# InternLM/lmdeploy

Measured on AMD Instinct MI355X. Metric: decode tokens/sec, Llama-3-8B W4A16 int8-KV batch 64 (1024-in/1k-out synthetic), higher is better.
Workload: dtype f16

## Files before the change

lmdeploy_amd/csrc/gemm_decode_lc.hip:

```cpp
#include "gemm_decode_common.h"
#include <stdlib.h>

namespace tmk {

typedef float floatx2 __attribute__((ext_vector_type(2)));

__device__ __forceinline__ half8_t raw8_p32(uint32_t w)
{
    const uint32_t m = 0x000f000fu;
    return bit_cast<half8_t>(u32x4{w & m, (w >> 4) & m, (w >> 8) & m, (w >> 12) & m});
}

template<int MH, int PFS, int ABL = 0>
__global__ __launch_bounds__(768) void gemm_dec_lc_kernel(Dec32Params p)
{
    constexpr int NCW   = 2;
    constexpr int CGW   = 2;
    constexpr int WK    = 4;
    constexpr int NCONS = CGW * WK;
    constexpr int NLOAD = 4;
    constexpr int T     = (NCONS + NLOAD) * 64;
    constexpr int ROWS  = 32 * MH;
    constexpr int KBB   = ROWS * 256;
    constexpr int S     = WK;
    constexpr int STG   = S * KBB;
    constexpr int CGT   = CGW * NCW;
    constexpr int NPC   = S * ROWS / 4;
    constexpr int DR    = NPC / NLOAD;
    static_assert(NPC % NLOAD == 0, "DMA pieces per loader wave");
    static_assert(WK * ROWS * CGT * 128 <= 2 * STG, "reduction image must fit the stage buffers");

    extern __shared__ __attribute__((aligned(16))) char smem[];

    const int tid  = threadIdx.x;
    const int wgid = blockIdx.y * gridDim.x + blockIdx.x;
    if (p.dbg && tid == 0) {
        p.dbg[wgid * 8 + 0] = __builtin_amdgcn_s_memrealtime();
        p.dbg[wgid * 8 + 4] = ((uint64_t)__builtin_amdgcn_s_getreg(20 | (31 << 11)) << 32) | (uint32_t)__builtin_amdgcn_s_getreg(4 | (31 << 11));
    }
    const int lane = tid & 63;
    const int wave = __builtin_amdgcn_readfirstlane(tid >> 6);
    const int l31  = lane & 31;
    const int half = lane >> 5;

    const int kb0 = blockIdx.y * p.kb_per_split;
    const int nkb = min(p.kb_per_split, p.KB - kb0);
    const int nst = (nkb + S - 1) / S;
    const int Mloc = min(ROWS, p.M);

    const unsigned lds0 = __builtin_amdgcn_readfirstlane((unsigned)(size_t)smem);

    floatx16 acc[NCW][MH];
#pragma unroll
    for (int c = 0; c < NCW; ++c) {
#pragma unroll
        for (int h = 0; h < MH; ++h) {
#pragma unroll
            for (int r = 0; r < 16; ++r) {
                acc[c][h][r] = 0.f;
            }
        }
    }
    const int cw = wave & (CGW - 1);
    const int wk = wave / CGW;

    if (wave >= NCONS) {
        const int  lw   = wave - NCONS;
        const auto rs_x = __builtin_amdgcn_make_buffer_rsrc((void*)p.x, 0, (int)(((size_t)(Mloc - 1) * p.ldx + p.K) * 2), 0x00020000);
        int        doff[DR];
#pragma unroll
        for (int r = 0; r < DR; ++r) {
            const int pc  = r * NLOAD + lw;
            const int kbi = pc / (ROWS / 4);
            const int row = (pc % (ROWS / 4)) * 4 + (lane >> 4);
            const int ch  = (lane & 15) ^ (row & 15);
            doff[r]       = (ABL & 0x20) ? (kbi * ROWS + row) * 256 + ch * 16
                                          : (min(row, Mloc - 1) * p.ldx + ch * 8) * 2 + kbi * 256;
        }
#define LC_DMA_X(t, buf)                                                                                          \
    _Pragma("unroll") for (int r = 0; r < DR; ++r)                                                                \
    {                                                                                                             \
        unsigned       keep_;                                                                                     \
        const unsigned dst_ = lds0 + (buf)*STG + (r * NLOAD + lw) * 1024;                                         \
        const int      so_  = (kb0 + (t)*S) * ((ABL & 0x20) ? ROWS * 256 : 256);                                  \
        asm volatile("s_mov_b32 %0, m0\n\ts_mov_b32 m0, %3\n\ts_nop 0\n\t"                                       \
                     "buffer_load_dwordx4 %1, %2, %4 offen lds\n\ts_mov_b32 m0, %0"                               \
                     : "=&s"(keep_)                                                                               \
                     : "v"(doff[r]), "s"(rs_x), "s"(dst_), "s"(so_)                                               \
                     : "memory");                                                                                 \
    }
        if (nst > 0) {
            if constexpr (!(ABL & 8)) {
                LC_DMA_X(0, 0);
            }
            asm volatile("s_waitcnt vmcnt(0)" ::: "memory");
            __builtin_amdgcn_s_barrier();
            for (int t = 0; t < nst; ++t) {
                if constexpr (!(ABL & 8)) {
                    if (t + 1 < nst) {
                        LC_DMA_X(t + 1, (t + 1) & 1);
                    }
                }
                asm volatile("s_waitcnt vmcnt(0)" ::: "memory");
                __builtin_amdgcn_s_barrier();
            }
        }
#undef LC_DMA_X
    }
    else {
        int cgc[NCW];
#pragma unroll
        for (int c = 0; c < NCW; ++c) {
            cgc[c] = min((int)blockIdx.x * CGT + cw * NCW + c, p.ncg - 1);
        }
        const auto rs_w = __builtin_amdgcn_make_buffer_rsrc((void*)p.wp, 0, (int)((size_t)p.KB * p.ncg * kP32Unit), 0x00020000);
        const int  vw   = lane * 16;
        const int  vs   = 2048 + l31 * 4;
        u32x4      ring[PFS][NCW][2];
        uint32_t   sring[PFS][NCW];
        const int frow = l31 * 256;
        const int fsw  = (half ^ (l31 & 15)) << 4;
        uint32_t  m1024 = 0x64006400u, m64 = 0x54005400u;
        asm volatile("" : "+v"(m1024), "+v"(m64));

#define LC_LOAD_W(slot, b)                                                                                        \
    _Pragma("unroll") for (int c = 0; c < NCW; ++c)                                                               \
    {                                                                                                             \
        const int uo_      = ((kb0 + min((b), nkb - 1)) * p.ncg + cgc[c]) * kP32Unit;                             \
        ring[slot][c][0]   = __builtin_amdgcn_raw_buffer_load_b128(rs_w, vw, uo_,  2);                      \
        ring[slot][c][1]   = __builtin_amdgcn_raw_buffer_load_b128(rs_w, vw + 1024, uo_,  2);               \
        sring[slot][c]     = __builtin_amdgcn_raw_buffer_load_b32(rs_w, vs, uo_, 0);                              \
    }
        if (nst > 0) {
#pragma unroll
            for (int u = 0; u < PFS; ++u) {
                if constexpr (!(ABL & 16)) {
                    LC_LOAD_W(u, u * S + wk);
                }
                __builtin_amdgcn_sched_barrier(0);
            }
            __builtin_amdgcn_s_barrier();
            if (p.dbg && tid == 0) {
                p.dbg[wgid * 8 + 1] = __builtin_amdgcn_s_memrealtime();
                p.dbg[wgid * 8 + 5] = __builtin_amdgcn_s_memtime();
            }
            auto stage = [&](auto U, const int t) __attribute__((always_inline)) {
                constexpr int u    = decltype(U)::value;
                const int     b    = t * S + wk;
                const bool    live = b < nkb;
                half2_t       s2[NCW], z2[NCW];
#pragma unroll
                for (int c = 0; c < NCW; ++c) {
                    const half2_t pr = bit_cast<half2_t>(live ? sring[u][c] : 0u);
                    s2[c]            = half2_t{pr[0], pr[0]};
                    z2[c]            = half2_t{pr[1], pr[1]};
                }
                half8_t        f0[MH], f1[MH];
                const unsigned xa = lds0 + (t & 1) * STG + wk * KBB;
                auto           rd = [&](half8_t(&f)[MH], int j) __attribute__((always_inline)) {
                    const unsigned ad = xa + (unsigned)(frow + ((32 * j) ^ fsw));
#pragma unroll
                    for (int h = 0; h < MH; ++h) {
                        asm volatile("ds_read_b128 %0, %1 offset:%2" : "=v"(f[h]) : "v"(ad), "i"(h * 8192));
                    }
                };
                auto wt = [&](half8_t(&f)[MH], auto N) __attribute__((always_inline)) {
                    constexpr int n = decltype(N)::value;
                    if constexpr (MH == 1) {
                        asm volatile("s_waitcnt lgkmcnt(%1)" : "+v"(f[0]) : "i"(n));
                    }
                    else {
                        asm volatile("s_waitcnt lgkmcnt(%2)" : "+v"(f[0]), "+v"(f[1]) : "i"(n));
                    }
                    __builtin_amdgcn_sched_barrier(0);
                };
                if constexpr (!(ABL & 4)) {
                    rd(f0, 0);
                }
                half8_t a0 = (ABL & 0x40) ? raw8_p32(ring[u][0][0][0]) : dequant8_p32(ring[u][0][0][0], s2[0], z2[0], m1024, m64), a1;
                if constexpr (ABL & 0x80) {
#pragma unroll
                    for (int c = 0; c < NCW; ++c) {
                        const float   rt = 1.0f + (float)s2[c][0];
                        const floatx2 rr = {rt, rt};
#pragma unroll
                        for (int h = 0; h < MH; ++h) {
#pragma unroll
                            for (int r = 0; r < 8; ++r) {
                                floatx2 v        = {acc[c][h][2 * r], acc[c][h][2 * r + 1]};
                                v                = v * rr;
                                acc[c][h][2 * r] = v[0], acc[c][h][2 * r + 1] = v[1];
                            }
                        }
                    }
                }
                static_for<8>([&](auto J) {
                    constexpr int  j  = decltype(J)::value;
                    half8_t(&cur)[MH] = (j & 1) ? f1 : f0;
                    half8_t(&nxt)[MH] = (j & 1) ? f0 : f1;
                    if constexpr (!(ABL & 4)) {
                        if constexpr (j + 1 < 8) {
                            rd(nxt, j + 1);
                        }
                        wt(cur, std::integral_constant<int, (j + 1 < 8) ? MH : 0>{});
                    }
                    else {
#pragma unroll
                        for (int h = 0; h < MH; ++h) {
                            cur[h] = bit_cast<half8_t>(ring[u][h & 1][1]);
                        }
                    }
                    if constexpr (ABL & 1) {
                        a1 = bit_cast<half8_t>(ring[u][1][j >> 2]);
                    }
                    else if constexpr (ABL & 0x40) {
                        a1 = raw8_p32(ring[u][1][j >> 2][j & 3]);
                    }
                    else {
                        a1 = dequant8_p32(ring[u][1][j >> 2][j & 3], s2[1], z2[1], m1024, m64);
                    }
#pragma unroll
                    for (int h = 0; h < MH; ++h) {
                        if constexpr (ABL & 2) {
                            asm volatile("" ::"v"(a0), "v"(cur[h]));
                        }
                        else {
                            acc[0][h] = __builtin_amdgcn_mfma_f32_32x32x16_f16(a0, cur[h], acc[0][h], 0, 0, 0);
                        }
                    }
                    if constexpr (j + 1 < 8) {
                        if constexpr (ABL & 1) {
                            a0 = bit_cast<half8_t>(ring[u][0][(j + 1) >> 2]);
                        }
                        else if constexpr (ABL & 0x40) {
                            a0 = raw8_p32(ring[u][0][(j + 1) >> 2][(j + 1) & 3]);
                        }
                        else {
                            a0 = dequant8_p32(ring[u][0][(j + 1) >> 2][(j + 1) & 3], s2[0], z2[0], m1024, m64);
                        }
                    }
#pragma unroll
                    for (int h = 0; h < MH; ++h) {
                        if constexpr (ABL & 2) {
                            asm volatile("" ::"v"(a1), "v"(cur[h]));
                        }
                        else {
                            acc[1][h] = __builtin_amdgcn_mfma_f32_32x32x16_f16(a1, cur[h], acc[1][h], 0, 0, 0);
                        }
                    }
                    if constexpr (!(ABL & (1 | 2))) {
#pragma unroll
                        for (int g = 0; g < 2 * MH; ++g) {
                            __builtin_amdgcn_sched_group_barrier(0x008, 1, 0);
                            __builtin_amdgcn_sched_group_barrier(0x002, MH == 2 ? 7 : 14, 0);
                        }
                    }
                    __builtin_amdgcn_sched_barrier(0);
                });
                if constexpr (!(ABL & 16)) {
                    LC_LOAD_W(u, (t + PFS) * S + wk);
                }
                __builtin_amdgcn_s_barrier();
            };
            int t0 = 0;
            for (; t0 + PFS <= nst; t0 += PFS) {
                static_for<PFS>([&](auto U) { stage(U, t0 + decltype(U)::value); });
            }
            static_for<PFS>([&](auto U) {
                if (t0 + decltype(U)::value < nst) {
                    stage(U, t0 + decltype(U)::value);
                }
            });
        }
#undef LC_LOAD_W
    }
    if (p.dbg && tid == 0) {
        p.dbg[wgid * 8 + 2] = __builtin_amdgcn_s_memrealtime();
        p.dbg[wgid * 8 + 6] = __builtin_amdgcn_s_memtime();
    }

    {
        constexpr int C4  = CGT * 8;
        floatx4*      red = (floatx4*)smem;
        if (wave < NCONS) {
#pragma unroll
            for (int c = 0; c < NCW; ++c) {
#pragma unroll
                for (int h = 0; h < MH; ++h) {
                    const int m = 32 * h + l31;
#pragma unroll
                    for (int g4 = 0; g4 < 4; ++g4) {
                        const int c4 = (cw * NCW + c) * 8 + 2 * g4 + half;
                        red[(wk * ROWS + m) * C4 + (c4 ^ (m & 7))] =
                            floatx4{acc[c][h][4 * g4], acc[c][h][4 * g4 + 1], acc[c][h][4 * g4 + 2], acc[c][h][4 * g4 + 3]};
                    }
                }
            }
        }
        __syncthreads();
        if (p.dbg && tid == 0) {
            p.dbg[wgid * 8 + 7] = __builtin_amdgcn_s_memrealtime();
        }
        constexpr int NE    = ROWS * C4;
        const int     ncol0 = blockIdx.x * CGT * 32;
#pragma unroll
        for (int e0 = 0; e0 < NE; e0 += T) {
            const int e = e0 + tid;
            if (NE % T != 0 && e >= NE) {
                break;
            }
            const int m  = e / C4;
            const int c4 = e % C4;
            floatx4   a  = red[m * C4 + (c4 ^ (m & 7))];
#pragma unroll
            for (int k = 1; k < WK; ++k) {
                a += red[(k * ROWS + m) * C4 + (c4 ^ (m & 7))];
            }
            const int n = ncol0 + c4 * 4;
            if (m >= Mloc || n >= p.N) {
                continue;
            }
            if (p.epilogue == 2) {
                floatx4* dst = (floatx4*)(p.partial + ((size_t)blockIdx.y * p.M + m) * p.N + n);
                if (p.wt & 1) {
                    store_wt(dst, a, p.wt >> 4);
                }
                else {
                    *dst = a;
                }
            }
            else if (p.epilogue == 1) {
                const float s0 = a[0] / (1.0f + __builtin_expf(-a[0]));
                const float s1 = a[2] / (1.0f + __builtin_expf(-a[2]));
                half2_t     o  = {(half_t)(s0 * a[1]), (half_t)(s1 * a[3])};
                half2_t*    dst = (half2_t*)(p.y + (size_t)m * p.ldy + (n >> 1));
                if (p.wt & 2) {
                    store_wt(dst, o);
                }
                else {
                    *dst = o;
                }
            }
            else {
                half4_t  o   = {(half_t)a[0], (half_t)a[1], (half_t)a[2], (half_t)a[3]};
                half4_t* dst = (half4_t*)(p.y + (size_t)m * p.ldy + n);
                if (p.wt & 2) {
                    store_wt(dst, o);
                }
                else {
                    *dst = o;
                }
            }
        }
    }
    if (p.dbg && tid == 0) {
        asm volatile("s_waitcnt vmcnt(0)" ::: "memory");
        p.dbg[wgid * 8 + 3] = __builtin_amdgcn_s_memrealtime();
    }
}

template<int MH, int PFS, int ABL = 0>
static int launch_lc_one(const Dec32Params& p, dim3 grid, hipStream_t st)
{
    constexpr int lds = 2 * 4 * 32 * MH * 256;
    if (const int rc = ensure_dynamic_lds((const void*)gemm_dec_lc_kernel<MH, PFS, ABL>, lds)) {
        return rc;
    }
    gemm_dec_lc_kernel<MH, PFS, ABL><<<grid, 768, lds, st>>>(p);
    TM_HIP_CHECK(hipGetLastError());
    return 0;
}

int launch_dec_lc(const Dec32Params& p, dim3 grid, hipStream_t st)
{
    static const int pfs = []() {
        const char* v = getenv("TM_LC_PFS");
        return v ? atoi(v) : 3;
    }();
#ifdef TM_EXPERIMENTS
    static const int abl = []() {
        const char* v = getenv("TM_D32_ABL");
        return v ? atoi(v) : -1;
    }();
    if (p.M > 32) {
        switch (abl) {
#define LC_CASE(v) case v: return launch_lc_one<2, 3, v>(p, grid, st)
            LC_CASE(0x20); LC_CASE(0x40); LC_CASE(0xc0); LC_CASE(0xe0); LC_CASE(1); LC_CASE(2); LC_CASE(4); LC_CASE(8); LC_CASE(16); LC_CASE(7); LC_CASE(15); LC_CASE(24); LC_CASE(31);
#undef LC_CASE
            default: break;
        }
    }
#endif
    if (p.M <= 32) {
        return pfs == 4 ? launch_lc_one<1, 4>(p, grid, st) : pfs == 2 ? launch_lc_one<1, 2>(p, grid, st) : launch_lc_one<1, 3>(p, grid, st);
    }
    return pfs == 4 ? launch_lc_one<2, 4>(p, grid, st) : pfs == 2 ? launch_lc_one<2, 2>(p, grid, st) : launch_lc_one<2, 3>(p, grid, st);
}

}
```

Baseline: 20360.

## Spread stage-0 activation DMA across consumer waves and batch reduction reads

The first stage's activation DMA into LDS is now split across all waves: consumer waves issue part of the pieces right after their first weight prefetch, and loader waves issue only the remainder. The goal is to shorten the prologue latency before the main loop starts. Consumers then wait on a vmcnt that still allows their outstanding weight loads to be in flight. The reduction epilogue is also restructured so that all LDS partial sums are read and accumulated first, then stored in a separate pass, letting the LDS reads overlap. This adds some register pressure and carries a risk if the vmcnt count is miscounted.

```diff
diff --git a/lmdeploy_amd/csrc/gemm_decode_lc.hip b/lmdeploy_amd/csrc/gemm_decode_lc.hip
--- a/lmdeploy_amd/csrc/gemm_decode_lc.hip
+++ b/lmdeploy_amd/csrc/gemm_decode_lc.hip
@@ -27,7 +27,10 @@
     constexpr int CGT   = CGW * NCW;
     constexpr int NPC   = S * ROWS / 4;
     constexpr int DR    = NPC / NLOAD;
+    constexpr int CP    = NPC / (NCONS + NLOAD);
+    constexpr int LP    = (NPC - NCONS * CP) / NLOAD;
     static_assert(NPC % NLOAD == 0, "DMA pieces per loader wave");
+    static_assert(NCONS * CP + NLOAD * LP == NPC, "stage 0 pieces over all waves");
     static_assert(WK * ROWS * CGT * 128 <= 2 * STG, "reduction image must fit the stage buffers");
 
     extern __shared__ __attribute__((aligned(16))) char smem[];
@@ -64,34 +67,44 @@
     const int cw = wave & (CGW - 1);
     const int wk = wave / CGW;
 
+    const auto rs_x = __builtin_amdgcn_make_buffer_rsrc((void*)p.x, 0, (int)(((size_t)(Mloc - 1) * p.ldx + p.K) * 2), 0x00020000);
+    auto x_off = [&](const int pc) __attribute__((always_inline)) {
+        const int kbi = pc / (ROWS / 4);
+        const int row = (pc % (ROWS / 4)) * 4 + (lane >> 4);
+        const int ch  = (lane & 15) ^ (row & 15);
+        return (ABL & 0x20) ? (kbi * ROWS + row) * 256 + ch * 16
+                            : (min(row, Mloc - 1) * p.ldx + ch * 8) * 2 + kbi * 256;
+    };
+    auto x_dma = [&](const int off, const int pc, const int t, const int buf) __attribute__((always_inline)) {
+        unsigned       keep;
+        const unsigned dst = lds0 + buf * STG + pc * 1024;
+        const int      so  = (kb0 + t * S) * ((ABL & 0x20) ? ROWS * 256 : 256);
+        asm volatile("s_mov_b32 %0, m0\n\ts_mov_b32 m0, %3\n\ts_nop 0\n\t"
+                     "buffer_load_dwordx4 %1, %2, %4 offen lds\n\ts_mov_b32 m0, %0"
+                     : "=&s"(keep)
+                     : "v"(off), "s"(rs_x), "s"(dst), "s"(so)
+                     : "memory");
+    };
+
     if (wave >= NCONS) {
-        const int  lw   = wave - NCONS;
-        const auto rs_x = __builtin_amdgcn_make_buffer_rsrc((void*)p.x, 0, (int)(((size_t)(Mloc - 1) * p.ldx + p.K) * 2), 0x00020000);
-        int        doff[DR];
+        const int lw = wave - NCONS;
+        int       doff[DR];
 #pragma unroll
         for (int r = 0; r < DR; ++r) {
-            const int pc  = r * NLOAD + lw;
-            const int kbi = pc / (ROWS / 4);
-            const int row = (pc % (ROWS / 4)) * 4 + (lane >> 4);
-            const int ch  = (lane & 15) ^ (row & 15);
-            doff[r]       = (ABL & 0x20) ? (kbi * ROWS + row) * 256 + ch * 16
-                                          : (min(row, Mloc - 1) * p.ldx + ch * 8) * 2 + kbi * 256;
+            doff[r] = x_off(r * NLOAD + lw);
         }
 #define LC_DMA_X(t, buf)                                                                                          \
     _Pragma("unroll") for (int r = 0; r < DR; ++r)                                                                \
     {                                                                                                             \
-        unsigned       keep_;                                                                                     \
-        const unsigned dst_ = lds0 + (buf)*STG + (r * NLOAD + lw) * 1024;                                         \
-        const int      so_  = (kb0 + (t)*S) * ((ABL & 0x20) ? ROWS * 256 : 256);                                  \
-        asm volatile("s_mov_b32 %0, m0\n\ts_mov_b32 m0, %3\n\ts_nop 0\n\t"                                       \
-                     "buffer_load_dwordx4 %1, %2, %4 offen lds\n\ts_mov_b32 m0, %0"                               \
-                     : "=&s"(keep_)                                                                               \
-                     : "v"(doff[r]), "s"(rs_x), "s"(dst_), "s"(so_)                                               \
-                     : "memory");                                                                                 \
+        x_dma(doff[r], r * NLOAD + lw, (t), (buf));                                                               \
     }
         if (nst > 0) {
             if constexpr (!(ABL & 8)) {
-                LC_DMA_X(0, 0);
+#pragma unroll
+                for (int r = 0; r < LP; ++r) {
+                    const int pc = NCONS * CP + lw + NLOAD * r;
+                    x_dma(x_off(pc), pc, 0, 0);
+                }
             }
             asm volatile("s_waitcnt vmcnt(0)" ::: "memory");
             __builtin_amdgcn_s_barrier();
@@ -138,6 +151,19 @@
                     LC_LOAD_W(u, u * S + wk);
                 }
                 __builtin_amdgcn_sched_barrier(0);
+                if constexpr (!(ABL & 8)) {
+                    if (u == 0) {
+#pragma unroll
+                        for (int r = 0; r < CP; ++r) {
+                            const int pc = wave + NCONS * r;
+                            x_dma(x_off(pc), pc, 0, 0);
+                        }
+                        __builtin_amdgcn_sched_barrier(0);
+                    }
+                }
+            }
+            if constexpr (!(ABL & 8)) {
+                asm volatile("s_waitcnt vmcnt(%0)" ::"i"((ABL & 16) ? 0 : (PFS - 1) * NCW * 3) : "memory");
             }
             __builtin_amdgcn_s_barrier();
             if (p.dbg && tid == 0) {
@@ -302,22 +328,27 @@
             p.dbg[wgid * 8 + 7] = __builtin_amdgcn_s_memrealtime();
         }
         constexpr int NE    = ROWS * C4;
+        constexpr int NI    = (NE + T - 1) / T;
+        static_assert(T % C4 == 0, "a pass covers whole rows");
         const int     ncol0 = blockIdx.x * CGT * 32;
-#pragma unroll
-        for (int e0 = 0; e0 < NE; e0 += T) {
-            const int e = e0 + tid;
-            if (NE % T != 0 && e >= NE) {
-                break;
-            }
-            const int m  = e / C4;
-            const int c4 = e % C4;
-            floatx4   a  = red[m * C4 + (c4 ^ (m & 7))];
+        floatx4 av[NI];
+#pragma unroll
+        for (int it = 0; it < NI; ++it) {
+            const int e = min(it * T + tid, NE - 1), m = e / C4, c4 = e % C4;
+            av[it]      = red[m * C4 + (c4 ^ (m & 7))];
 #pragma unroll
             for (int k = 1; k < WK; ++k) {
-                a += red[(k * ROWS + m) * C4 + (c4 ^ (m & 7))];
-            }
-            const int n = ncol0 + c4 * 4;
-            if (m >= Mloc || n >= p.N) {
+                av[it] += red[(k * ROWS + m) * C4 + (c4 ^ (m & 7))];
+            }
+        }
+#pragma unroll
+        for (int it = 0; it < NI; ++it) {
+            const int     e  = it * T + tid;
+            const int     m  = e / C4;
+            const int     c4 = e % C4;
+            const floatx4 a  = av[it];
+            const int     n  = ncol0 + c4 * 4;
+            if (e >= NE || m >= Mloc || n >= p.N) {
                 continue;
             }
             if (p.epilogue == 2) {
```

Result: no change. 20280 (-0.4%).
